# tsai0507/PolishPathPlanning

Hardware: AMD Instinct MI355X
Metric: polishing waypoints/sec for 1M-pt cloud, 256 slices; path L2 err vs ref (higher is better)
Workload: dtype f32; 1 GPU; cfg2_1m_s256; points_per_workpiece=999912, slices=256, waypoints_per_workpiece=25908, workpieces=1, batch_per_gpu=1, parallelism=single GPU, pairing=kd, walk=center_int (connect), dynamic_adjustment=False, handles_taking_turns=3

## Files before the change

polishpathplanning_amd/csrc/ppp_engine.hip:

```cpp
#include "ppp_kernels.h"
#ifdef PPP_SINGLE_TU
#include "ppp_window.h"
#endif
#include "ppp_handle.h"
#include "ppp_gather.h"
#include <atomic>
#include <cerrno>
#include <fcntl.h>
#include <thread>
#include <unistd.h>
#ifndef PPP_NN_HINT_SPACINGS
#define PPP_NN_HINT_SPACINGS 3.0
#endif
#ifndef PPP_SLAB_PTS
#define PPP_SLAB_PTS 832
#endif
#ifndef PPP_PPT8_FROM
#define PPP_PPT8_FROM 500000
#endif
#ifndef WIN_SLICE_WAVES_PER_CU
#define WIN_SLICE_WAVES_PER_CU 16
#endif
#ifndef PPP_WIN_PPT8_FROM
#define PPP_WIN_PPT8_FROM 1200000
// ... 373 lines not shown
        fprintf(stderr, "[ppp] window plan: S %d [%d,%d) pad %.2f capw %d cap_el %d NBc %d (throughput %d) threads %d ppt %d x %d threads lds %zu B max window %d max left side %d census %s\n",
                S, h->sb, h->se, pad, capw, cap_el, NBc, h->win_NBc_thr, T, h->win_ppt, h->win_scat_threads, win_slice_lds_for(h, NBc), max_w, max_el,
                from_auto ? "came with the cloud" : (inherit ? "inherited from an earlier cloud of this size" : "at plan time"));
    return PPP_OK;
}

static WinArgs win_args(const ppp_handle h)
{
    WinArgs A;
    memset(&A, 0, sizeof(A));
    A.m = h->meta.p; A.P = dev_params(h);
    A.X = h->use_part ? h->Xp.p : h->X.p; A.Y = h->use_part ? h->Yp.p : h->Y.p; A.Z = h->use_part ? h->Zp.p : h->Z.p;
    A.idmap = h->use_part ? h->part_idx.p : ((h->part_given && h->part_has_idx) ? h->part_idx.p : nullptr);
    A.n = h->use_part ? h->n_part : (int)h->n;
    A.plan_px = h->win_px.p;
    A.S = h->S_cap; A.sb = h->sb; A.se = h->se; A.first_kept = h->win_first_kept; A.nkept = h->win_nkept;
    A.pad = h->win_pad; A.px0 = h->win_px0; A.inv_step = 1.0f / (float)std::max(1, (int)(h->P.tool_radius * 2));
    A.y0 = h->h_mn[1];
    { const float yr = h->h_mx[1] - h->h_mn[1]; A.yscale = yr > 0.f ? (float)h->win_NBc / yr : 0.f; }
    for (int d = 0; d < 3; ++d) { A.plan_mn[d] = h->h_mn[d]; A.plan_mx[d] = h->h_mx[d]; }
    A.plan_nvalid = h->h_nvalid;
    A.capw = h->win_capw; A.cap_el = h->win_cap_el; A.NB = h->win_NB; A.NBc = h->win_NBc; A.stride = h->win_stride; A.rec_lds = h->win_rec_lds;
    A.W_cap = h->W_cap; A.node_cap = h->node_cap;
    A.g_scatter = h->win_gs; A.g_slice = std::max(0, h->se - h->sb); A.g_finish = h->sm_tiles;
    A.finish = h->ranged ? 0 : 1;
    A.win_cnt = h->win_cnt.p; A.win_pts = h->win_pts.p; A.win_part = h->win_part.p;
    A.px = h->px.p; A.lo = h->lo.p; A.hi = h->hi.p;
    A.node_x = h->node_x.p; A.node_y = h->node_y.p; A.node_z = h->node_z.p;
    A.node_start = h->node_start.p; A.node_cnt = h->node_cnt.p; A.band_cnt = h->band_cnt.p;
    A.wp_cnt = h->wp_cnt.p; A.wp_off = h->wp_off.p; A.tail = h->tail.p;
    A.wps_xyz = h->wps_xyz.p; A.wps_normal = h->wps_normal.p; A.wps_nn = h->wps_nn.p; A.wps_pre = h->wps_pre.p; A.wps_rec = h->wps_rec.p;
    A.wp_pre = h->wp_pre.p; A.wp_smooth = h->wp_smooth.p; A.wp_out = h->wp_out.p; A.out2 = h->out2; A.out2_cap = h->out2_cap;
    A.plan_rec = (h->rec_current && h->plan_walk_ok) ? h->plan_auto.p : nullptr;
    A.meta_host = h->hmeta_pinned.p; A.fin_ticket = h->fin_ticket.p;
    return A;
}
static size_t win_slice_lds(const ppp_handle h) { return win_slice_lds_for(h, h->win_NBc); }
static void win_args_throughput(const ppp_handle h, WinArgs &A)
{
    A.NBc = h->win_NBc_thr; A.NB = WIN_CLASSES * A.NBc;
    const float yr = h->h_mx[1] - h->h_mn[1];
    A.yscale = yr > 0.f ? (float)A.NBc / yr : 0.f;
}

static int enqueue_window_gen(ppp_handle h)
{
    WinArgs A = win_args(h);
    const bool thr = win_throughput_launch(h, A.g_slice);
    if (thr) win_args_throughput(h, A);
    const size_t scat_lds = win_scatter_lds_bytes(A.S, h->win_ppt, h->win_scat_threads, h->win_staged);
    if (h->win_scat_threads != WSC_T) {
        const int rcn = with_narrow_scatter(h->win_scat_threads, h->win_ppt, [&](auto ppt, auto st) -> int {
            LAUNCH(h, "k_win_scatter", (k_win_scatter<decltype(ppt)::value, false, decltype(st)::value>), A.g_scatter, decltype(st)::value, scat_lds, A);
            return PPP_OK;
        });
        if (rcn) return rcn;
    }
    else if (h->win_staged && h->win_ppt == 8) LAUNCH(h, "k_win_scatter", (k_win_scatter<8, true>), A.g_scatter, WSC_T, scat_lds, A);
    else if (h->win_staged) LAUNCH(h, "k_win_scatter", (k_win_scatter<4, true>), A.g_scatter, WSC_T, scat_lds, A);
    else if (h->win_ppt == 8) LAUNCH(h, "k_win_scatter", (k_win_scatter<8, false>), A.g_scatter, WSC_T, scat_lds, A);
    else if (h->win_ppt == 2) LAUNCH(h, "k_win_scatter", (k_win_scatter<2, false>), A.g_scatter, WSC_T, scat_lds, A);
    else LAUNCH(h, "k_win_scatter", (k_win_scatter<4, false>), A.g_scatter, WSC_T, scat_lds, A);
    const int T = h->win_threads;
    const size_t lds = win_slice_lds_for(h, A.NBc);
    const int extra = tuning_env("PPP_WIN_NO_VERIFY") ? 0 : 1;
    return with_block_size(T, [&](auto bs) -> int {
        LAUNCH(h, "k_win_slice", k_win_slice<decltype(bs)::value>, A.g_slice + extra, T, lds, A);
// ... 580 lines not shown
extern "C" {

void ppp_default_params(ppp_params *p)
{
    memset(p, 0, sizeof(*p));
    p->tool_radius = 12; p->path_resolution = 7; p->rpy_resolution = 7; p->ee_length = 0.3f;
    p->change_range = 1; p->pairing = PPP_PAIR_KD; p->walk = PPP_WALK_CENTER_INT;
    p->trim = 10; p->drop_ends = 1; p->smooth = 1;
    const float he[6] = {-0.764091f, 0.025886f, 0.663790f, -3.1270175f, -0.040124f, -1.6063578f};
    memcpy(p->handeye, he, sizeof(he));
    p->normal_radius = 2.5f;
    p->smooth_max_sweeps = 32;
    p->alignment = 0; p->dynamic_adjustment = 0;
    p->depth = 0.01; p->adjust_threshold = 1; p->toolthickness = 10; p->curvature_k = 50;
    p->slice_begin = 0; p->slice_end = 0; p->range_margin = 24.f;
}

const char *ppp_version(void) { return PPP_VERSION_STR; }

int ppp_create(int device_id, ppp_handle *out)
{
    if (!out) return PPP_ERR_ARG;
    *out = nullptr;
    int count = 0;
    if (hipGetDeviceCount(&count) != hipSuccess || count <= 0) return PPP_ERR_NO_DEVICE;
    if (device_id < 0 || device_id >= count) return PPP_ERR_ARG;
    if (hipSetDevice(device_id) != hipSuccess) return PPP_ERR_HIP;
    ppp_handle h = new ppp_handle_s();
    h->device = device_id;
    ppp_default_params(&h->P);
    if (hipStreamCreateWithFlags(&h->stream, hipStreamNonBlocking) != hipSuccess) { delete h; return PPP_ERR_HIP; }
    if (h->meta.ensure(1) != hipSuccess) { delete h; return PPP_ERR_HIP; }
    if (hipMemset(h->meta.p, 0, sizeof(DevMeta)) != hipSuccess) { delete h; return PPP_ERR_HIP; }
    if (h->fin_ticket.ensure(1 + WIN_FIN_GROUPS) != hipSuccess || hipMemset(h->fin_ticket.p, 0, sizeof(int) * (1 + WIN_FIN_GROUPS)) != hipSuccess) { delete h; return PPP_ERR_HIP; }
    if (h->hmeta_pinned.ensure(1) != hipSuccess) { delete h; return PPP_ERR_HIP; }
    int lds = 0;
    if (hipDeviceGetAttribute(&lds, hipDeviceAttributeMaxSharedMemoryPerBlock, device_id) == hipSuccess && lds > 0) h->max_lds = lds;
    hipDeviceProp_t prop;
    if (hipGetDeviceProperties(&prop, device_id) == hipSuccess) {
        if (strncmp(prop.gcnArchName, "gfx950", 6) == 0) h->max_lds = std::max(h->max_lds, 160 * 1024);
        if (prop.multiProcessorCount > 0) h->num_cus = prop.multiProcessorCount;
    }
    (void)hipFuncSetAttribute((const void *)k_slice, hipFuncAttributeMaxDynamicSharedMemorySize, h->max_lds - 1024);
    (void)hipFuncSetAttribute((const void *)k_slice_kd<false>, hipFuncAttributeMaxDynamicSharedMemorySize, h->max_lds - 1024);
    (void)hipFuncSetAttribute((const void *)k_minmax<true>, hipFuncAttributeMaxDynamicSharedMemorySize, 16384 * 4);
    (void)hipFuncSetAttribute((const void *)k_slab_scatter<1, 8>, hipFuncAttributeMaxDynamicSharedMemorySize, 16384 * 4);
    (void)hipFuncSetAttribute((const void *)k_slab_scatter<2, 4>, hipFuncAttributeMaxDynamicSharedMemorySize, 16384 * 4);
    (void)hipFuncSetAttribute((const void *)k_minmax_b, hipFuncAttributeMaxDynamicSharedMemorySize, 16384 * 4);
    (void)hipFuncSetAttribute((const void *)k_slab_scatter_b<4>, hipFuncAttributeMaxDynamicSharedMemorySize, 16384 * 4);
    (void)hipFuncSetAttribute((const void *)k_slab_scatter_b<8>, hipFuncAttributeMaxDynamicSharedMemorySize, 16384 * 4);
    (void)hipFuncSetAttribute((const void *)k_scatter_setup<4>, hipFuncAttributeMaxDynamicSharedMemorySize, 16384 * 4);
    (void)hipFuncSetAttribute((const void *)k_scatter_setup<8>, hipFuncAttributeMaxDynamicSharedMemorySize, 16384 * 4);
    (void)hipFuncSetAttribute((const void *)k_scatter_setup<16>, hipFuncAttributeMaxDynamicSharedMemorySize, 16384 * 4);
    (void)hipFuncSetAttribute((const void *)k_slice_kd_b, hipFuncAttributeMaxDynamicSharedMemorySize, h->max_lds - 1024);
    (void)hipFuncSetAttribute((const void *)k_pose_b<256>, hipFuncAttributeMaxDynamicSharedMemorySize, h->max_lds - 8192);
    (void)hipFuncSetAttribute((const void *)k_pose_b<512>, hipFuncAttributeMaxDynamicSharedMemorySize, h->max_lds - 8192);
    (void)hipFuncSetAttribute((const void *)k_pose_b<768>, hipFuncAttributeMaxDynamicSharedMemorySize, h->max_lds - 8192);
    (void)hipFuncSetAttribute((const void *)k_pose_b<POSE_T>, hipFuncAttributeMaxDynamicSharedMemorySize, h->max_lds - 8192);
    (void)hipFuncSetAttribute((const void *)k_pose<false, 256>, hipFuncAttributeMaxDynamicSharedMemorySize, h->max_lds - 8192);
    (void)hipFuncSetAttribute((const void *)k_pose<false, 512>, hipFuncAttributeMaxDynamicSharedMemorySize, h->max_lds - 8192);
    (void)hipFuncSetAttribute((const void *)k_pose<false, 768>, hipFuncAttributeMaxDynamicSharedMemorySize, h->max_lds - 8192);
    (void)hipFuncSetAttribute((const void *)k_pose<false, POSE_T>, hipFuncAttributeMaxDynamicSharedMemorySize, h->max_lds - 8192);
    (void)hipFuncSetAttribute((const void *)k_pose<true, POSE_T>, hipFuncAttributeMaxDynamicSharedMemorySize, h->max_lds - 8192);
    (void)hipFuncSetAttribute((const void *)k_dyn_boundary_pts, hipFuncAttributeMaxDynamicSharedMemorySize, 152 * 1024);
    (void)hipFuncSetAttribute((const void *)k_dyn_adjust_pts, hipFuncAttributeMaxDynamicSharedMemorySize, 152 * 1024);
    (void)hipFuncSetAttribute((const void *)k_dyn_adjust_fit, hipFuncAttributeMaxDynamicSharedMemorySize, 96 * 1024);
    (void)hipFuncSetAttribute((const void *)k_band_indices, hipFuncAttributeMaxDynamicSharedMemorySize, h->max_lds - 1024);
// ... 1476 lines not shown
```

polishpathplanning_amd/csrc/ppp_handle.h:

```cpp
#pragma once
#include "ppp_window_decl.h"
#include "ppp_dynamic.h"
#include "ppp_compact.h"
#include "../../include/ppp_hip.h"
#include <algorithm>
#include <cmath>
#include <cstdlib>
#include <functional>
#include <memory>
#include <string>
#include <vector>

struct RegAcc;
struct FeedRec;

namespace ppp_internal __attribute__((visibility("hidden"))) {

struct KTimer {
    std::string name;
    std::vector<hipEvent_t> e0, e1;
    int used = 0;
};

template <typename T, bool PINNED>
// ... 264 lines not shown
        int source = -1;
        float threshold = 0.f, link = 0.f;
        unsigned long long serial = 0;
        ppp_region_stats stats = {};
    } regions;
    DevBuf<int> node_start, node_cnt, band_cnt;
    DevBuf<int> wp_cnt, wp_off, tail, slice_wpcnt;
    DevBuf<float4> wp_xyz, wp_normal;
    DevBuf<int> wp_nn;
    DevBuf<float> wp_pre, wp_smooth, wp_out;
    DevBuf<MinMaxPart> mm_part;
    DevBuf<int> big_slabs, big_slices;
    DevBuf<char> arena;
    bool big_path = false;
    int mm_grid = 1, sm_tiles = 1;
    DevBuf<char> scratch;
    bool win_allowed = true;
    bool win_disabled = false;
    bool win_path = false;
    bool win_staged = false;
    float win_pad = 4.f;
    int win_NBc_thr = 0;
    int win_capw = 0, win_cap_el = 0, win_NB = 0, win_NBc = 0, win_stride = 1, win_threads = 256, win_ppt = 4, win_gs = 1;
    int win_scat_threads = WSC_T;
    int win_ppt_alone = 4;
    int win_rec_lds = 0;
    int win_nkept = 0, win_first_kept = 0, win_el_expect = 0;
    float win_px0 = 0.f;
    DevBuf<float> win_px;
    DevBuf<int> win_cnt;
    DevBuf<float4> win_pts;
    DevBuf<MinMaxPart> win_part;
    DevBuf<float4> wps_xyz, wps_normal, wps_rec;
    DevBuf<int> fin_ticket;
    DevBuf<int> wps_nn;
    DevBuf<float> wps_pre;

    DevMeta hmeta;
    PinBuf<DevMeta> hmeta_pinned;
    DevBuf<int> plan_ticket;
    DevBuf<PlanAuto> plan_auto;
    bool auto_valid = false;
    bool plan_reuse = true;
    bool inh_valid = false;
    int inh_S = 0, inh_n = 0, inh_max_w = 0, inh_max_el = 0;
    float inh_pad = 0.f;
    ppp_params inh_P;
    bool auto_px_only = false;
    bool plan_inherited = false;
    int auto_S = 0;
    float auto_pad = 0.f;
    bool slab_cnt_used = true;
    PinBuf<char> pin;
    PinBuf<char> pcd_stage[2];
    hipEvent_t pcd_ev[2] = {nullptr, nullptr};
    int side_by_side = 1;
    bool plan_deferred = false, deferred_census = false;
    bool rec_current = false;
    bool plan_walk_ok = false;
    bool chain_calls = false;
    float *out2 = nullptr;
    int out2_cap = 0;
    float *last_out2 = nullptr;
    int last_out2_cap = 0;
    int internal = 0;
    hipGraph_t graph = nullptr;
    hipGraphExec_t graph_exec = nullptr;
// ... 161 lines not shown
```

polishpathplanning_amd/csrc/ppp_window.h:

```cpp
#pragma once
#include "ppp_kernels.h"
#include "ppp_window_decl.h"

template <int PPT, bool STAGED, int T = WSC_T>
__device__ __forceinline__ void win_scatter_body(const WinArgs &A, const int bx)
{
    extern __shared__ __attribute__((aligned(16))) int s_dyn[];
    float *s_px = (float *)s_dyn;
    int *s_cnt = s_dyn + A.S;
    __shared__ int s_scr[17];
    __shared__ float s_mn[3][T / 64], s_mx[3][T / 64];
    __shared__ int s_n[T / 64];
    const int S = A.S, n = A.n;
    const int i0 = bx * (PPT * (int)blockDim.x);
    STAMP_BEGIN();
    float4 p[PPT];
#pragma unroll
    for (int k = 0; k < PPT; ++k) {
        const int i = i0 + threadIdx.x + k * (int)blockDim.x;
        if (i < n) p[k] = make_float4(A.X[i], A.Y[i], A.Z[i], __int_as_float(A.idmap ? A.idmap[i] : i));
        else p[k] = make_float4(NAN, 0.f, 0.f, 0.f);
    }
    for (int s = threadIdx.x; s < S; s += blockDim.x) { s_px[s] = A.plan_px[s]; s_cnt[s] = 0; }
    if (bx == 0 && threadIdx.x == 0) {
        DevMeta *m = A.m;
        m->W = 0; m->err = 0; m->err_slice = 0x7fffffff; m->sweeps = 0; m->any_short = 0; m->rpy_oob = 0;
        m->node_cursor = 0; m->smooth_done = -1; m->emit_ticket = 0; m->big_slabs = 0; m->big_slices = 0; m->arena_cursor = 0; m->win_flag = 0;
        if (A.fin_ticket) for (int q = 0; q <= WIN_FIN_GROUPS; ++q) A.fin_ticket[q] = 0;
    }
    __syncthreads();
    STAMP(7, 0);
    float mn[3] = {INFINITY, INFINITY, INFINITY}, mx[3] = {-INFINITY, -INFINITY, -INFINITY};
    int cnt = 0;
    constexpr bool PACKED = PPT >= 16;
    static_assert(!PACKED || (T * PPT <= 65536 && WIN_S_MAX <= 32768), "window and rank share a word");
    int pw[PPT], pr[PACKED ? 1 : PPT];
    auto put = [&](int k, int w, int r) { if constexpr (PACKED) pw[k] = (w << 16) | r; else { pw[k] = w; pr[k] = r; } };
    auto win_of = [&](int k) -> int { if constexpr (PACKED) return pw[k] >> 16; else return pw[k]; };
    auto rank_of = [&](int k) -> int { if constexpr (PACKED) return pw[k] & 0xffff; else return pr[k]; };
#pragma unroll
    for (int k = 0; k < PPT; ++k) {
        const float x = p[k].x;
        pw[k] = -1; if constexpr (!PACKED) pr[k] = 0;
        if (x == x) {
            mn[0] = fminf(mn[0], x); mx[0] = fmaxf(mx[0], x);
            mn[1] = fminf(mn[1], p[k].y); mx[1] = fmaxf(mx[1], p[k].y);
            mn[2] = fminf(mn[2], p[k].z); mx[2] = fmaxf(mx[2], p[k].z);
            cnt++;
            const float fj = fminf(fmaxf(floorf((x - s_px[0]) * A.inv_step + 0.5f), 0.f), (float)(S - 1));
            const int j = (int)fj;
            const int ja = j > 0 ? j - 1 : j, jb = j + 1 < S ? j + 1 : j;
            const float da = fabsf(x - s_px[ja]), dj = fabsf(x - s_px[j]), db = fabsf(x - s_px[jb]);
            int w = -1;
            if (dj <= A.pad) w = j; else if (da <= A.pad) w = ja; else if (db <= A.pad) w = jb;
            if (w >= A.sb && w < A.se) {
                put(k, w, atomicAdd(&s_cnt[w], 1));
            }
        }
    }
    __syncthreads();
    STAMP(7, 1);
// ... 60 lines not shown
        for (int w = 0; w < nw; ++w) r.cnt += s_n[w];
        for (int d = 0; d < 3; ++d) {
            float a = INFINITY, b = -INFINITY;
            for (int w = 0; w < nw; ++w) { a = fminf(a, s_mn[d][w]); b = fmaxf(b, s_mx[d][w]); }
            r.mn[d] = a; r.mx[d] = b;
        }
        A.win_part[bx] = r;
    }
    STAMP(7, 4);
}

__device__ __forceinline__ void win_lds_barrier() { asm volatile("s_waitcnt lgkmcnt(0)\n\ts_barrier" ::: "memory"); }

template <int PPT>
__device__ __forceinline__ void win_scatter_staged_loop(const WinArgs &A, const int bx, const int nwg)
{
    extern __shared__ __attribute__((aligned(16))) int s_dyn[];
    float *s_px = (float *)s_dyn;
    int *s_cnt = s_dyn + A.S;
    __shared__ int s_scr[17];
    __shared__ float s_mn[3][WSC_T / 64], s_mx[3][WSC_T / 64];
    __shared__ int s_n[WSC_T / 64];
    const int S = A.S, n = A.n, T = (int)blockDim.x;
    const int chunk_pts = PPT * T;
    const int nchunks = (n + chunk_pts - 1) / chunk_pts;
    int *s_loc = (int *)s_px;
    int *s_gb = s_dyn + 2 * S;
    float4 *stage = (float4 *)(s_dyn + ((3 * S + 3) & ~3));
    u16 *widx = (u16 *)(stage + PPT * T);
    if (bx == 0 && threadIdx.x == 0) {
        DevMeta *m = A.m;
        m->W = 0; m->err = 0; m->err_slice = 0x7fffffff; m->sweeps = 0; m->any_short = 0; m->rpy_oob = 0;
        m->node_cursor = 0; m->smooth_done = -1; m->emit_ticket = 0; m->big_slabs = 0; m->big_slices = 0; m->arena_cursor = 0; m->win_flag = 0;
        if (A.fin_ticket) for (int q = 0; q <= WIN_FIN_GROUPS; ++q) A.fin_ticket[q] = 0;
    }
    float4 p[PPT], pn[PPT];
    auto request = [&](int chunk, float4 *dst) {
        const int i0 = chunk * chunk_pts;
#pragma unroll
        for (int k = 0; k < PPT; ++k) {
            const int i = i0 + (int)threadIdx.x + k * T;
            if (i < n) dst[k] = make_float4(A.X[i], A.Y[i], A.Z[i], __int_as_float(A.idmap ? A.idmap[i] : i));
            else dst[k] = make_float4(NAN, 0.f, 0.f, 0.f);
        }
    };
    if (bx < nchunks) request(bx, p);
    float mn[3] = {INFINITY, INFINITY, INFINITY}, mx[3] = {-INFINITY, -INFINITY, -INFINITY};
    int cnt = 0;
    for (int chunk = bx; chunk < nchunks; chunk += nwg) {
        for (int s = threadIdx.x; s < S; s += T) { s_px[s] = A.plan_px[s]; s_cnt[s] = 0; }
        __syncthreads();
        int pw[PPT], pr[PPT];
#pragma unroll
        for (int k = 0; k < PPT; ++k) {
            const float x = p[k].x;
            pw[k] = -1; pr[k] = 0;
            if (x == x) {
                mn[0] = fminf(mn[0], x); mx[0] = fmaxf(mx[0], x);
                mn[1] = fminf(mn[1], p[k].y); mx[1] = fmaxf(mx[1], p[k].y);
                mn[2] = fminf(mn[2], p[k].z); mx[2] = fmaxf(mx[2], p[k].z);
                cnt++;
                const float fj = fminf(fmaxf(floorf((x - s_px[0]) * A.inv_step + 0.5f), 0.f), (float)(S - 1));
                const int j = (int)fj;
                const int ja = j > 0 ? j - 1 : j, jb = j + 1 < S ? j + 1 : j;
                const float da = fabsf(x - s_px[ja]), dj = fabsf(x - s_px[j]), db = fabsf(x - s_px[jb]);
                int w = -1;
                if (dj <= A.pad) w = j; else if (da <= A.pad) w = ja; else if (db <= A.pad) w = jb;
// ... 732 lines not shown
            for (int d = 0; d < 3; ++d) if (rmn[d] != R.fin.mn[d] || rmx[d] != R.fin.mx[d]) bad = 1;
            if (c != R.fin.cnt || R.S != A.S || __float_as_int(R.pad) != __float_as_int(A.pad)) bad = 1;
        } else {
            for (int d = 0; d < 3; ++d) if (rmn[d] != A.plan_mn[d] || rmx[d] != A.plan_mx[d]) bad = 1;
            if (c != A.plan_nvalid) bad = 1;
        }
        int S = c ? slice_walk_device(P.walk, rmn[0], rmx[0], P.tool_radius, s_px, A.S, s_front, 2048) : 0;
        if (S != A.S) bad = 1;
        for (int d = 0; d < 3; ++d) { m->mn[d] = rmn[d]; m->mx[d] = rmx[d]; m->mn_ord[d] = f2ord(rmn[d]); m->mx_ord[d] = f2ord(rmx[d]); }
        m->n_valid = c;
        m->S = S > A.S ? A.S : S;
        m->first_kept = P.drop_ends ? 1 : 0;
        { const int Sc = S > A.S ? A.S : S, nk = P.drop_ends ? Sc - 2 : Sc; m->nkept = nk < 0 ? 0 : nk; }
        m->sb = A.sb; m->se = A.se;
        m->incl_lo = P.incl_lo; m->incl_hi = P.incl_hi;
        s_S = S > A.S ? A.S : S;
        if (bad) s_bad = 1;
    }
    __syncthreads();
    const int S = s_S;
    int bad = 0;
    for (int s = tid; s < S; s += T) {
        const float v = s_px[s];
        if (v != A.plan_px[s]) bad = 1;
        const int position = (int)v;
        A.px[s] = v; A.lo[s] = (float)(-2 + position); A.hi[s] = (float)(2 + position);
    }
    if (bad) s_bad = 1;
    __syncthreads();
    if (tid == 0 && s_bad) win_flag(m, WIN_FLAG_STALE);
}

#define META_PUT(ptr, val) __hip_atomic_store((ptr), (val), __ATOMIC_RELAXED, __HIP_MEMORY_SCOPE_AGENT)
template <bool ONDEMAND>
__device__ __forceinline__ void win_finish_body(const WinArgs &A, const int bx)
{
    extern __shared__ __attribute__((aligned(16))) int s_off[];
    __shared__ float s_x[3][SMF_M];
    __shared__ int s_scan[17];
    __shared__ int s_run, s_short, s_last, s_err;
    __shared__ double s_rp[SMF_END];
    __shared__ double s_e[2][3];
    DevMeta *m = A.m;
    const DevParams &P = A.P;
    const int nk = A.nkept, tid = (int)threadIdx.x;
    const int res_i = (int)P.rpy_resolution;
    int W;
    if (nk <= 4 * SMF_T) {
        int c4[4];
#pragma unroll
        for (int u = 0; u < 4; ++u) {
            const int k2 = 4 * tid + u, s2 = k2 + A.first_kept;
            c4[u] = (k2 < nk && s2 >= A.sb && s2 < A.se) ? A.wp_cnt[k2] : 0;
        }
        if (tid == 0) { s_err = m->err | m->win_flag; s_short = 0; }
        int tot;
        int pre = block_exscan_w(c4[0] + c4[1] + c4[2] + c4[3], s_scan, &tot);
        if (s_err) return;
        bool shrt = false;
#pragma unroll
        for (int u = 0; u < 4; ++u) {
            const int k2 = 4 * tid + u;
            if (k2 < nk) {
                s_off[k2] = pre;
                pre += c4[u];
                if (c4[u] <= res_i) shrt = true;
            }
        }
        if (P.rpy_resolution > 2 && shrt) s_short = 1;
        W = tot;
    } else {
        if (tid == 0) { s_err = m->err | m->win_flag; s_run = 0; s_short = 0; }
        __syncthreads();
        if (s_err) return;
        for (int base = 0; base < nk; base += blockDim.x) {
            const int k2 = base + tid;
            int c2 = 0;
            if (k2 < nk) {
                const int s2 = k2 + A.first_kept;
                if (s2 >= A.sb && s2 < A.se) c2 = A.wp_cnt[k2];
            }
            int tot;
            const int pre = block_exscan_w(c2, s_scan, &tot);
            const int run = s_run;
            if (k2 < nk) {
                s_off[k2] = run + pre;
                if (P.rpy_resolution > 2 && c2 <= res_i) s_short = 1;
            }
            __syncthreads();
            if (tid == 0) s_run = run + tot;
            __syncthreads();
        }
        W = s_run;
    }
    if (tid == 0) s_off[nk] = W;
    __syncthreads();
    if (W > A.W_cap) { if (!ONDEMAND && bx == 0 && tid == 0) { set_err(m, DERR_CAPACITY, -1); META_PUT(&m->W, 0); } return; }
    if (!ONDEMAND && bx == 0) {
        for (int k2 = tid; k2 < nk; k2 += blockDim.x) {
            A.wp_off[k2] = s_off[k2]; A.tail[k2] = s_off[k2 + 1] - 1;
            const int s2 = k2 + A.first_kept;
            if (s2 < A.sb || s2 >= A.se) A.wp_cnt[k2] = 0;
        }
        if (tid == 0) { A.wp_off[nk] = W; META_PUT(&m->W, W); META_PUT(&m->any_short, s_short); META_PUT(&m->sweeps, 0); META_PUT(&m->smooth_done, 0); }
    }
    const int ntiles = smooth_tiles(W);
    const int tile = bx;
    if (W == 0 || tile >= ntiles) return;
    auto slice_of = [&](int g) {
        int kk = (int)(((long long)g * (long long)nk) / (long long)W);
        kk = kk < 0 ? 0 : (kk > nk - 1 ? nk - 1 : kk);
        int steps = 0;
        while (kk > 0 && s_off[kk] > g && steps < 6) { --kk; ++steps; }
        while (kk < nk - 1 && s_off[kk + 1] <= g && steps < 6) { ++kk; ++steps; }
        if (steps >= 6) { int lo = 0, hi = nk - 1; while (lo < hi) { const int mid = (lo + hi + 1) >> 1; if (s_off[mid] <= g) lo = mid; else hi = mid - 1; } kk = lo; }
        return kk;
    };
    auto row_of = [&](int g) { const int kk = slice_of(g); return (size_t)kk * A.stride + (size_t)(g - s_off[kk]); };
    const double wd = 0.65, ws = 1 - wd, dg = wd + 2 * ws;
    const double r = (dg - sqrt(dg * dg - 4 * ws * ws)) / (2 * ws), c = wd / (dg - 2 * ws * r);
    const int t0 = tile * SMF_T;
    const int base = t0 - SMF_K;
    const bool solve = A.finish && P.smooth && W > 2;
    const bool in_order = A.finish && P.rpy_resolution > 2 && s_short;
    const bool lists = ONDEMAND || A.stage_lists || !A.finish || in_order;
    const bool near_end = solve && (t0 < SMF_END || t0 + SMF_T - 1 > W - 1 - SMF_END);
    const int g = t0 + tid;
    int kk = 0;
    size_t rowbase = 0;
    if (g < W) {
        kk = slice_of(g);
        rowbase = (size_t)kk * A.stride - (size_t)s_off[kk];
    }
    const bool halo = A.finish && tid < 2 * SMF_K;
    const int hl = tid < SMF_K ? tid : SMF_T + tid;
    bool hsrc = false;
    size_t hrow = 0;
    if (halo) {
        const int g2 = base + hl;
        hsrc = g2 >= 1 && g2 <= W - 2;
        if (hsrc) hrow = row_of(g2);
// ... 14 lines not shown
    }
    const int ej = tid >> 6, lane = tid & 63;
    const bool eterm = near_end && ej < 3;
    const int kq = (lane & 31) + 1;
    bool qsrc = false;
    size_t qrow = 0, erow = 0;
    if (eterm) {
        const int gq = lane < 32 ? kq : W - 1 - kq;
        qsrc = gq >= 1 && gq <= W - 2;
        if (qsrc) qrow = row_of(gq);
        if ((lane & 31) == 0) erow = row_of(lane < 32 ? 0 : W - 1);
    }
    typedef const __attribute__((address_space(1))) float *gfloat_p;
    const gfloat_p wps = (gfloat_p)A.wps_pre;
    const size_t orow = g < W ? rowbase + (size_t)g : 0;
    const int ejc = ej < 3 ? ej : 0;
    float p[6], hx[3], ka[3], kb[3];
#pragma unroll
    for (int d = 0; d < 6; ++d) p[d] = wps[6 * orow + d];
#pragma unroll
    for (int j = 0; j < 3; ++j) hx[j] = wps[6 * hrow + j];
#pragma unroll
    for (int D = 3; D < 6; ++D) kb[D - 3] = wps[6 * krow_b + D];
#pragma unroll
    for (int D = 3; D < 6; ++D) ka[D - 3] = wps[6 * krow_a + D];
    const float qv = wps[6 * qrow + ejc], ev = wps[6 * erow + ejc];
    if (A.finish) {
        const bool src = g >= 1 && g <= W - 2;
        for (int j = 0; j < 3; ++j) s_x[j][tid + SMF_K] = src ? p[j] : 0.f;
        const int hslot = halo ? hl : tid + SMF_K;
        for (int j = 0; j < 3; ++j) s_x[j][hslot] = halo ? (hsrc ? hx[j] : 0.f) : (src ? p[j] : 0.f);
    }
    const bool copy2 = !ONDEMAND && A.finish && A.out2 != nullptr && W <= A.out2_cap;
    if (!ONDEMAND && A.finish && A.out2 != nullptr && W > A.out2_cap && tile == 0 && tid == 0) set_err(m, DERR_CAPACITY, -1);
    if (near_end) {
        if (tid < SMF_END) s_rp[tid] = smooth_rpow(r, tid);
        if (ej < 3) {
            double v = qsrc ? (double)qv * smooth_rpow(r, kq) : 0.0;
            for (int o = 16; o > 0; o >>= 1) v += __shfl_xor(v, o, 64);
            if ((lane & 31) == 0) s_e[lane >> 5][ej] = (double)ev - c * v;
        }
    }
    __syncthreads();
    if (g < W) {
#pragma clang fp contract(on)
        if (lists) for (int d = 0; d < 6; ++d) A.wp_pre[6 * (size_t)g + d] = p[d];
        if (A.finish) {
            if (solve) {
                const int l = g - base;
                double acc[3], y[3];
#pragma unroll
                for (int j = 0; j < 3; ++j) acc[j] = (double)s_x[j][l - SMF_K] + (double)s_x[j][l + SMF_K];
#pragma unroll 8
                for (int q = SMF_K - 1; q >= 1; --q) {
#pragma unroll
                    for (int j = 0; j < 3; ++j) acc[j] = ((double)s_x[j][l - q] + (double)s_x[j][l + q]) + r * acc[j];
                }
#pragma unroll
                for (int j = 0; j < 3; ++j) y[j] = c * ((double)s_x[j][l] + r * acc[j]);
                if (near_end) {
                    const double D = W - 1 < SMF_END ? s_rp[W - 1] : 0.0;
                    const double r0 = g < SMF_END ? s_rp[g] : 0.0, r1 = W - 1 - g < SMF_END ? s_rp[W - 1 - g] : 0.0;
                    const double det = 1.0 - D * D;
#pragma unroll
                    for (int j = 0; j < 3; ++j) {
                        const double e0 = s_e[0][j], e1 = s_e[1][j];
                        const double Aa = (e0 - D * e1) / det, Bb = (e1 - D * e0) / det;
// ... 22 lines not shown
                                    dr = (double)fabsf(a - bb) < fabs(no1 - no2) ? (double)(a - bb) : (no1 - no2);
                                    dr /= res;
                                }
                                float v = bb;
                                for (int q = 1; q <= wi; ++q) v = (float)(dr + v);
                                p[D] = v;
                            }
                        }
                        for (int D = 3; D < 6; ++D) p[D] = (double)p[D] > M_PI ? (float)((double)p[D] - 2 * M_PI) : p[D];
                    }
                    float R[3][3];
                    rot_zyx(p[3], p[4], p[5], R);
                    const float ee[3] = {0.f, 0.f, -P.ee_length};
                    float t[3];
                    for (int i = 0; i < 3; ++i) t[i] = R[i][0] * ee[0] + R[i][1] * ee[1] + R[i][2] * ee[2] + p[i] * 1.f;
                    p[0] = t[0]; p[1] = t[1]; p[2] = t[2];
                }
                for (int d = 0; d < 6; ++d) A.wp_out[6 * (size_t)g + d] = p[d];
                if (copy2 && !in_order) for (int d = 0; d < 6; ++d) A.out2[6 * (size_t)g + d] = p[d];
            }
        }
    }
    if (!ONDEMAND && in_order) {
        __threadfence();
        __syncthreads();
        if (tid == 0) s_last = atomicAdd(&m->emit_ticket, 1) == ntiles - 1;
        __syncthreads();
        if (s_last) {
            __threadfence();
            if (tid == 0) { finish_list_in_order(m, P, A.tail, A.wp_out); m->emit_ticket = 0; }
            __threadfence();
            __syncthreads();
            if (copy2) for (size_t i = tid; i < 6 * (size_t)W; i += blockDim.x) A.out2[i] = A.wp_out[i];
        }
    }
}

__global__ void __launch_bounds__(256) k_win_gather_stage(WinArgs A, float4 *wp_xyz, int *wp_nn, float4 *wp_normal)
{
    const int k = blockIdx.x;
    if (k >= A.nkept) return;
    const int s = k + A.first_kept;
    if (s < A.sb || s >= A.se) return;
    const int off = A.wp_off[k], cnt = A.wp_cnt[k];
    for (int t = threadIdx.x; t < cnt; t += blockDim.x) {
        const size_t slot = (size_t)k * A.stride + t;
        wp_xyz[off + t] = A.wps_xyz[slot];
        wp_nn[off + t] = A.wps_nn[slot];
        wp_normal[off + t] = A.wps_normal[slot];
    }
}



__device__ __forceinline__ void win_census_point(float x, const float *__restrict__ px, int S, float px0, float inv_step, float pad,
                                                 int *cw, int *ce, int *cr)
{
    if (!(x == x)) return;
    const float fj = fminf(fmaxf(floorf((x - px0) * inv_step + 0.5f), 0.f), (float)(S - 1));
    const int j = (int)fj;
    const int ja = j > 0 ? j - 1 : j, jb = j + 1 < S ? j + 1 : j;
    int w = -1;
    if (fabsf(x - px[j]) <= pad) w = j; else if (fabsf(x - px[ja]) <= pad) w = ja; else if (fabsf(x - px[jb]) <= pad) w = jb;
    if (w < 0) return;
    atomicAdd(&cw[w], 1);
    const float Px = px[w];
// ... 77 lines not shown
    }
}

template <int PPT, bool STAGED, int T>
__global__ void __launch_bounds__(T) k_win_scatter(WinArgs A)
{
    static_assert(!STAGED || T == WSC_T, "the staged form is one workgroup of WSC_T threads per CU");
    if (STAGED) win_scatter_staged_loop<PPT>(A, blockIdx.x, A.g_scatter);
    else win_scatter_body<PPT, false, T>(A, blockIdx.x);
}
template <int PPT, bool STAGED, int T>
__global__ void __launch_bounds__(T) k_win_scatter_b(const WinArgs *__restrict__ mem)
{
    static_assert(!STAGED || T == WSC_T, "the staged form is one workgroup of WSC_T threads per CU");
    const WinArgs &A = mem[blockIdx.y];
    if ((int)blockIdx.x >= A.g_scatter) return;
    if (STAGED) win_scatter_staged_loop<PPT>(A, blockIdx.x, A.g_scatter);
    else win_scatter_body<PPT, false, T>(A, blockIdx.x);
}
template <int TMAX>
__global__ void __launch_bounds__(TMAX) k_win_slice(WinArgs A)
{
    if ((int)blockIdx.x == A.g_slice) { win_verify_body(A); return; }
    win_slice_body<TMAX>(A, blockIdx.x);
}
template <int TMAX>
__global__ void __launch_bounds__(TMAX) k_win_slice_b(const WinArgs *__restrict__ mem)
{
    const WinArgs &A = mem[blockIdx.y];
    if ((int)blockIdx.x > A.g_slice) return;
    if ((int)blockIdx.x == A.g_slice) { win_verify_body(A); return; }
    win_slice_body<TMAX>(A, blockIdx.x);
}
__device__ __forceinline__ void win_publish_meta(const WinArgs &A)
{
    if (!A.meta_host) return;
    __shared__ int s_lastw;
    __syncthreads();
    if (threadIdx.x == 0) {
        __builtin_amdgcn_s_waitcnt(0);
        const int grp = (int)blockIdx.x % WIN_FIN_GROUPS;
        const int members = (A.g_finish - grp + WIN_FIN_GROUPS - 1) / WIN_FIN_GROUPS;
        int last = 0;
        if (__hip_atomic_fetch_add(A.fin_ticket + 1 + grp, 1, __ATOMIC_RELAXED, __HIP_MEMORY_SCOPE_AGENT) == members - 1) {
            __hip_atomic_store(A.fin_ticket + 1 + grp, 0, __ATOMIC_RELAXED, __HIP_MEMORY_SCOPE_AGENT);
            const int groups = A.g_finish < WIN_FIN_GROUPS ? A.g_finish : WIN_FIN_GROUPS;
            last = __hip_atomic_fetch_add(A.fin_ticket, 1, __ATOMIC_RELAXED, __HIP_MEMORY_SCOPE_AGENT) == groups - 1;
        }
        s_lastw = last;
    }
    __syncthreads();
    if (!s_lastw) return;
    const int *src = (const int *)A.m;
    int *dst = (int *)A.meta_host;
    for (int q = threadIdx.x; q < (int)(sizeof(DevMeta) / sizeof(int)); q += blockDim.x) dst[q] = __hip_atomic_load(src + q, __ATOMIC_RELAXED, __HIP_MEMORY_SCOPE_AGENT);
    if (threadIdx.x == 0) __hip_atomic_store(A.fin_ticket, 0, __ATOMIC_RELAXED, __HIP_MEMORY_SCOPE_AGENT);
}
__global__ void __launch_bounds__(SMF_T) k_win_finish(WinArgs A) { win_finish_body<false>(A, blockIdx.x); win_publish_meta(A); }
__global__ void __launch_bounds__(SMF_T) k_win_finish_b(const WinArgs *__restrict__ mem)
{
    const WinArgs &A = mem[blockIdx.y];
    if ((int)blockIdx.x >= A.g_finish) return;
    win_finish_body<false>(A, blockIdx.x);
    win_publish_meta(A);
}
__global__ void __launch_bounds__(SMF_T) k_win_stage_lists(WinArgs A) { win_finish_body<true>(A, blockIdx.x); }
```

polishpathplanning_amd/csrc/ppp_window_decl.h:

```cpp
#pragma once
#include "ppp_kernels.h"

enum { WIN_FLAG_OVERFLOW = 1,
       WIN_FLAG_REACH = 2,
       WIN_FLAG_STALE = 4 };
__device__ inline void win_flag(DevMeta *m, int why) { atomicOr(&m->win_flag, why); }

#define WIN_CLASSES 5
#ifndef WIN_CNT_STRIDE
#define WIN_CNT_STRIDE 1
#endif
#ifndef WIN_EMAX
#define WIN_EMAX 8
#endif
#ifndef WIN_CE
#define WIN_CE 4
#endif

struct WinArgs {
    DevMeta *m;
    DevParams P;
    const float *X, *Y, *Z;
    const int *idmap;
    int n;
    const float *plan_px;
    int S, sb, se, first_kept, nkept;
    float pad, px0, inv_step, y0, yscale;
    float plan_mn[3], plan_mx[3];
    int plan_nvalid;
    int capw, cap_el, NB, NBc, stride, W_cap, node_cap;
    int rec_lds;
    int g_scatter, g_slice, g_finish;
    int finish;
    int stage_lists;
    int *win_cnt;
    float4 *win_pts;
    MinMaxPart *win_part;
    float *px, *lo, *hi;
    float *node_x, *node_y, *node_z;
    int *node_start, *node_cnt, *band_cnt;
    int *wp_cnt, *wp_off, *tail;
    float4 *wps_xyz, *wps_normal;
    float4 *wps_rec;
    int *wps_nn;
    float *wps_pre;
    float *wp_pre, *wp_smooth, *wp_out, *out2;
    int out2_cap;
    DevMeta *meta_host;
    int *fin_ticket;
    const PlanAuto *plan_rec;
};

__host__ __device__ inline size_t win_slice_lds_bytes(int capw, int cap_el, int NB)
{
    return (size_t)capw * 16 + (((size_t)NB + 1) * 4 + 15) / 16 * 16 + (size_t)cap_el * 16 + 16;
}

#ifndef WSC_T
#define WSC_T 1024
#endif
__host__ __device__ inline size_t win_scatter_lds_bytes(int S, int ppt, int threads, bool staged)
{
    return staged ? (size_t)12 * S + 16 + (size_t)18 * ppt * threads : (size_t)8 * S;
}
#ifndef WSL_T
#define WSL_T 1024
#endif
#define WIN_FIN_GROUPS 32
#define WIN_S_MAX 8192
#define WIN_AUTO_SCAP 4096

template <int PPT, bool STAGED, int T = WSC_T> __global__ void k_win_scatter(WinArgs A);
template <int PPT, bool STAGED, int T = WSC_T> __global__ void k_win_scatter_b(const WinArgs *__restrict__ mem);
template <int TMAX> __global__ void k_win_slice(WinArgs A);
template <int TMAX> __global__ void k_win_slice_b(const WinArgs *__restrict__ mem);
__global__ void k_win_finish(WinArgs A);
__global__ void k_win_finish_b(const WinArgs *__restrict__ mem);
__global__ void k_win_stage_lists(WinArgs A);
__global__ void k_win_gather_stage(WinArgs A, float4 *wp_xyz, int *wp_nn, float4 *wp_normal);
template <bool IN_LDS>
__global__ void k_win_census(const float *__restrict__ X, int n, const float *__restrict__ px, int S, float px0, float inv_step, float pad,
                             int *cnt_win, int *cnt_el, int *cnt_er);
__global__ void k_win_census_auto(const float *__restrict__ X, int n, const float *px, const PlanAuto *plan, float inv_step, int *cnt, int *ticket,
                                  PlanAuto *plan_host, float *px_host, int *census_host);
```

Before: 979.0 million waypoints/s.

## Publish finish metadata to host from workgroup zero instead of ticket-counted last block

Removes the grouped atomic ticket scheme that found the last finishing workgroup to copy the device meta block to pinned host memory. Workgroup zero now loads the meta words up front, patches the fields it decides itself (W, any_short, sweeps, smooth_done, err), and writes them to host directly. The in-order smoothing path copies from memory at its end. This drops per-block atomics, waitcnt and extra barriers from every finish workgroup. The risk is that host-visible meta could miss updates made by other workgroups, such as errors set later.

```diff
diff --git a/polishpathplanning_amd/csrc/ppp_engine.hip b/polishpathplanning_amd/csrc/ppp_engine.hip
--- a/polishpathplanning_amd/csrc/ppp_engine.hip
+++ b/polishpathplanning_amd/csrc/ppp_engine.hip
@@ -429,7 +429,7 @@
     A.wps_xyz = h->wps_xyz.p; A.wps_normal = h->wps_normal.p; A.wps_nn = h->wps_nn.p; A.wps_pre = h->wps_pre.p; A.wps_rec = h->wps_rec.p;
     A.wp_pre = h->wp_pre.p; A.wp_smooth = h->wp_smooth.p; A.wp_out = h->wp_out.p; A.out2 = h->out2; A.out2_cap = h->out2_cap;
     A.plan_rec = (h->rec_current && h->plan_walk_ok) ? h->plan_auto.p : nullptr;
-    A.meta_host = h->hmeta_pinned.p; A.fin_ticket = h->fin_ticket.p;
+    A.meta_host = h->hmeta_pinned.p;
     return A;
 }
 static size_t win_slice_lds(const ppp_handle h) { return win_slice_lds_for(h, h->win_NBc); }
@@ -1076,7 +1076,6 @@
     if (hipStreamCreateWithFlags(&h->stream, hipStreamNonBlocking) != hipSuccess) { delete h; return PPP_ERR_HIP; }
     if (h->meta.ensure(1) != hipSuccess) { delete h; return PPP_ERR_HIP; }
     if (hipMemset(h->meta.p, 0, sizeof(DevMeta)) != hipSuccess) { delete h; return PPP_ERR_HIP; }
-    if (h->fin_ticket.ensure(1 + WIN_FIN_GROUPS) != hipSuccess || hipMemset(h->fin_ticket.p, 0, sizeof(int) * (1 + WIN_FIN_GROUPS)) != hipSuccess) { delete h; return PPP_ERR_HIP; }
     if (h->hmeta_pinned.ensure(1) != hipSuccess) { delete h; return PPP_ERR_HIP; }
     int lds = 0;
     if (hipDeviceGetAttribute(&lds, hipDeviceAttributeMaxSharedMemoryPerBlock, device_id) == hipSuccess && lds > 0) h->max_lds = lds;
diff --git a/polishpathplanning_amd/csrc/ppp_handle.h b/polishpathplanning_amd/csrc/ppp_handle.h
--- a/polishpathplanning_amd/csrc/ppp_handle.h
+++ b/polishpathplanning_amd/csrc/ppp_handle.h
@@ -320,7 +320,6 @@
     DevBuf<float4> win_pts;
     DevBuf<MinMaxPart> win_part;
     DevBuf<float4> wps_xyz, wps_normal, wps_rec;
-    DevBuf<int> fin_ticket;
     DevBuf<int> wps_nn;
     DevBuf<float> wps_pre;
 
diff --git a/polishpathplanning_amd/csrc/ppp_window.h b/polishpathplanning_amd/csrc/ppp_window.h
--- a/polishpathplanning_amd/csrc/ppp_window.h
+++ b/polishpathplanning_amd/csrc/ppp_window.h
@@ -26,7 +26,6 @@
         DevMeta *m = A.m;
         m->W = 0; m->err = 0; m->err_slice = 0x7fffffff; m->sweeps = 0; m->any_short = 0; m->rpy_oob = 0;
         m->node_cursor = 0; m->smooth_done = -1; m->emit_ticket = 0; m->big_slabs = 0; m->big_slices = 0; m->arena_cursor = 0; m->win_flag = 0;
-        if (A.fin_ticket) for (int q = 0; q <= WIN_FIN_GROUPS; ++q) A.fin_ticket[q] = 0;
     }
     __syncthreads();
     STAMP(7, 0);
@@ -153,7 +152,6 @@
         DevMeta *m = A.m;
         m->W = 0; m->err = 0; m->err_slice = 0x7fffffff; m->sweeps = 0; m->any_short = 0; m->rpy_oob = 0;
         m->node_cursor = 0; m->smooth_done = -1; m->emit_ticket = 0; m->big_slabs = 0; m->big_slices = 0; m->arena_cursor = 0; m->win_flag = 0;
-        if (A.fin_ticket) for (int q = 0; q <= WIN_FIN_GROUPS; ++q) A.fin_ticket[q] = 0;
     }
     float4 p[PPT], pn[PPT];
     auto request = [&](int chunk, float4 *dst) {
@@ -952,6 +950,20 @@
 }
 
 #define META_PUT(ptr, val) __hip_atomic_store((ptr), (val), __ATOMIC_RELAXED, __HIP_MEMORY_SCOPE_AGENT)
+#define META_WORDS ((int)(sizeof(DevMeta) / sizeof(int)))
+#define META_WORD(field) ((int)(offsetof(DevMeta, field) / sizeof(int)))
+static_assert(sizeof(DevMeta) % sizeof(int) == 0 && META_WORDS <= SMF_T, "a thread of the finish workgroup per word of the meta block");
+__device__ __forceinline__ void win_meta_to_host(const WinArgs &A, int word)
+{
+    if (A.meta_host && (int)threadIdx.x < META_WORDS) ((int *)A.meta_host)[threadIdx.x] = word;
+}
+__device__ __forceinline__ void win_meta_from_memory(const WinArgs &A)
+{
+    if (!A.meta_host) return;
+    const int *src = (const int *)A.m;
+    int *dst = (int *)A.meta_host;
+    for (int q = threadIdx.x; q < META_WORDS; q += blockDim.x) dst[q] = __hip_atomic_load(src + q, __ATOMIC_RELAXED, __HIP_MEMORY_SCOPE_AGENT);
+}
 template <bool ONDEMAND>
 __device__ __forceinline__ void win_finish_body(const WinArgs &A, const int bx)
 {
@@ -965,6 +977,9 @@
     const DevParams &P = A.P;
     const int nk = A.nkept, tid = (int)threadIdx.x;
     const int res_i = (int)P.rpy_resolution;
+    const bool wg0 = !ONDEMAND && bx == 0;
+    int mw = 0;
+    if (wg0) mw = __hip_atomic_load((const __attribute__((address_space(1))) int *)m + (tid < META_WORDS ? tid : 0), __ATOMIC_RELAXED, __HIP_MEMORY_SCOPE_AGENT);
     int W;
     if (nk <= 4 * SMF_T) {
         int c4[4];
@@ -976,7 +991,7 @@
         if (tid == 0) { s_err = m->err | m->win_flag; s_short = 0; }
         int tot;
         int pre = block_exscan_w(c4[0] + c4[1] + c4[2] + c4[3], s_scan, &tot);
-        if (s_err) return;
+        if (s_err) { if (wg0) win_meta_to_host(A, mw); return; }
         bool shrt = false;
 #pragma unroll
         for (int u = 0; u < 4; ++u) {
@@ -992,7 +1007,7 @@
     } else {
         if (tid == 0) { s_err = m->err | m->win_flag; s_run = 0; s_short = 0; }
         __syncthreads();
-        if (s_err) return;
+        if (s_err) { if (wg0) win_meta_to_host(A, mw); return; }
         for (int base = 0; base < nk; base += blockDim.x) {
             const int k2 = base + tid;
             int c2 = 0;
@@ -1015,7 +1030,11 @@
     }
     if (tid == 0) s_off[nk] = W;
     __syncthreads();
-    if (W > A.W_cap) { if (!ONDEMAND && bx == 0 && tid == 0) { set_err(m, DERR_CAPACITY, -1); META_PUT(&m->W, 0); } return; }
+    if (W > A.W_cap) {
+        if (!ONDEMAND && bx == 0 && tid == 0) { set_err(m, DERR_CAPACITY, -1); META_PUT(&m->W, 0); }
+        if (wg0) win_meta_to_host(A, tid == META_WORD(err) ? (int)DERR_CAPACITY : (tid == META_WORD(W) ? 0 : mw));
+        return;
+    }
     if (!ONDEMAND && bx == 0) {
         for (int k2 = tid; k2 < nk; k2 += blockDim.x) {
             A.wp_off[k2] = s_off[k2]; A.tail[k2] = s_off[k2 + 1] - 1;
@@ -1024,9 +1043,17 @@
         }
         if (tid == 0) { A.wp_off[nk] = W; META_PUT(&m->W, W); META_PUT(&m->any_short, s_short); META_PUT(&m->sweeps, 0); META_PUT(&m->smooth_done, 0); }
     }
+    auto decided = [&](bool refused) {
+        int w = mw;
+        if (tid == META_WORD(W)) w = W;
+        if (tid == META_WORD(any_short)) w = s_short;
+        if (tid == META_WORD(sweeps) || tid == META_WORD(smooth_done)) w = 0;
+        if (tid == META_WORD(err) && refused) w = DERR_CAPACITY;
+        return w;
+    };
     const int ntiles = smooth_tiles(W);
     const int tile = bx;
-    if (W == 0 || tile >= ntiles) return;
+    if (W == 0 || tile >= ntiles) { if (wg0) win_meta_to_host(A, decided(false)); return; }
     auto slice_of = [&](int g) {
         int kk = (int)(((long long)g * (long long)nk) / (long long)W);
         kk = kk < 0 ? 0 : (kk > nk - 1 ? nk - 1 : kk);
@@ -1107,7 +1134,9 @@
         for (int j = 0; j < 3; ++j) s_x[j][hslot] = halo ? (hsrc ? hx[j] : 0.f) : (src ? p[j] : 0.f);
     }
     const bool copy2 = !ONDEMAND && A.finish && A.out2 != nullptr && W <= A.out2_cap;
-    if (!ONDEMAND && A.finish && A.out2 != nullptr && W > A.out2_cap && tile == 0 && tid == 0) set_err(m, DERR_CAPACITY, -1);
+    const bool refuse2 = !ONDEMAND && A.finish && A.out2 != nullptr && W > A.out2_cap;
+    if (refuse2 && tile == 0 && tid == 0) set_err(m, DERR_CAPACITY, -1);
+    if (wg0 && !in_order) win_meta_to_host(A, decided(refuse2));
     if (near_end) {
         if (tid < SMF_END) s_rp[tid] = smooth_rpow(r, tid);
         if (ej < 3) {
@@ -1196,6 +1225,7 @@
             __threadfence();
             __syncthreads();
             if (copy2) for (size_t i = tid; i < 6 * (size_t)W; i += blockDim.x) A.out2[i] = A.wp_out[i];
+            win_meta_from_memory(A);
         }
     }
 }
@@ -1339,36 +1369,11 @@
     if ((int)blockIdx.x == A.g_slice) { win_verify_body(A); return; }
     win_slice_body<TMAX>(A, blockIdx.x);
 }
-__device__ __forceinline__ void win_publish_meta(const WinArgs &A)
-{
-    if (!A.meta_host) return;
-    __shared__ int s_lastw;
-    __syncthreads();
-    if (threadIdx.x == 0) {
-        __builtin_amdgcn_s_waitcnt(0);
-        const int grp = (int)blockIdx.x % WIN_FIN_GROUPS;
-        const int members = (A.g_finish - grp + WIN_FIN_GROUPS - 1) / WIN_FIN_GROUPS;
-        int last = 0;
-        if (__hip_atomic_fetch_add(A.fin_ticket + 1 + grp, 1, __ATOMIC_RELAXED, __HIP_MEMORY_SCOPE_AGENT) == members - 1) {
-            __hip_atomic_store(A.fin_ticket + 1 + grp, 0, __ATOMIC_RELAXED, __HIP_MEMORY_SCOPE_AGENT);
-            const int groups = A.g_finish < WIN_FIN_GROUPS ? A.g_finish : WIN_FIN_GROUPS;
-            last = __hip_atomic_fetch_add(A.fin_ticket, 1, __ATOMIC_RELAXED, __HIP_MEMORY_SCOPE_AGENT) == groups - 1;
-        }
-        s_lastw = last;
-    }
-    __syncthreads();
-    if (!s_lastw) return;
-    const int *src = (const int *)A.m;
-    int *dst = (int *)A.meta_host;
-    for (int q = threadIdx.x; q < (int)(sizeof(DevMeta) / sizeof(int)); q += blockDim.x) dst[q] = __hip_atomic_load(src + q, __ATOMIC_RELAXED, __HIP_MEMORY_SCOPE_AGENT);
-    if (threadIdx.x == 0) __hip_atomic_store(A.fin_ticket, 0, __ATOMIC_RELAXED, __HIP_MEMORY_SCOPE_AGENT);
-}
-__global__ void __launch_bounds__(SMF_T) k_win_finish(WinArgs A) { win_finish_body<false>(A, blockIdx.x); win_publish_meta(A); }
+__global__ void __launch_bounds__(SMF_T) k_win_finish(WinArgs A) { win_finish_body<false>(A, blockIdx.x); }
 __global__ void __launch_bounds__(SMF_T) k_win_finish_b(const WinArgs *__restrict__ mem)
 {
     const WinArgs &A = mem[blockIdx.y];
     if ((int)blockIdx.x >= A.g_finish) return;
     win_finish_body<false>(A, blockIdx.x);
-    win_publish_meta(A);
 }
 __global__ void __launch_bounds__(SMF_T) k_win_stage_lists(WinArgs A) { win_finish_body<true>(A, blockIdx.x); }
diff --git a/polishpathplanning_amd/csrc/ppp_window_decl.h b/polishpathplanning_amd/csrc/ppp_window_decl.h
--- a/polishpathplanning_amd/csrc/ppp_window_decl.h
+++ b/polishpathplanning_amd/csrc/ppp_window_decl.h
@@ -47,7 +47,6 @@
     float *wp_pre, *wp_smooth, *wp_out, *out2;
     int out2_cap;
     DevMeta *meta_host;
-    int *fin_ticket;
     const PlanAuto *plan_rec;
 };
 
@@ -66,7 +65,6 @@
 #ifndef WSL_T
 #define WSL_T 1024
 #endif
-#define WIN_FIN_GROUPS 32
 #define WIN_S_MAX 8192
 #define WIN_AUTO_SCAP 4096
 
```

Result: no change. 976.6 million waypoints/s (-0.2%).
